# pablomendes/kubeflow-tfx-workshop

Measured on AMD Instinct MI355X. Metric: Trainer examples/sec (whole node), Chicago-Taxi Wide&Deep at 1/2/4/8 MI355X, higher is better.
Workload: dtype bf16; 1 GPU; global_batch=65536, parallelism=dp1, batch_per_gpu=65536, optimizer=adagrad(dnn,lr=0.05)+ftrl(linear,lr=0.2), precision=bf16 MFMA compute, fp32 master weights/optimizer state, device=AMD Radeon Graphics, hipgraph=True, input_shuffle_seed=24301, steps_per_graph=20, kernel=wd_chain (register-chained, 8 waves)

## Files before the change

### csrc/wd_chain.hip

```cpp
#include <hip/hip_runtime.h>
#include "xcd.h"
#include "feed.h"
#include <stdint.h>

namespace {

typedef __bf16 bf16;
typedef __bf16 v8bf __attribute__((ext_vector_type(8)));
typedef __bf16 v4bf __attribute__((ext_vector_type(4)));
typedef __bf16 v2bf __attribute__((ext_vector_type(2)));
typedef short v4s __attribute__((ext_vector_type(4)));
typedef short v8s __attribute__((ext_vector_type(8)));
typedef float v4f __attribute__((ext_vector_type(4)));
typedef __attribute__((address_space(3))) v4s lds_v4s;

#include "wd_opt.h"

#ifndef WDC_T
#define WDC_T 128
#endif
constexpr int T = WDC_T;
static_assert(T == 128 || T == 64 || T == 256, "T");
constexpr bool ONE_ITER = T == 256 || T == 64;
constexpr int MAXW = 8;
constexpr int WPAD = 16;
constexpr int PAD = 8;

constexpr int K1 = 32, N1 = 128;
constexpr int K2 = 128, N2 = 96;
constexpr int K3 = 96, N3 = 64;
constexpr int K4 = 64, N4 = 64;
constexpr int K5 = 64, N5 = 16;

constexpr int LW1 = 0;
constexpr int LW2 = LW1 + N1 * (K1 + WPAD);
constexpr int LW3 = LW2 + N2 * (K2 + WPAD);
constexpr int LW4 = LW3 + N3 * (K3 + WPAD);
constexpr int LW5 = LW4 + N4 * (K4 + WPAD);
constexpr int LWEND = LW5 + N5 * (K5 + WPAD);
constexpr int stage_len(int K, int N) { return T * (N + PAD) + T * (K + PAD); }
constexpr int cmax(int a, int b) { return a > b ? a : b; }
constexpr int WIDE_PAD = 2176;
constexpr bool ROT = T == 256;
constexpr int DMA_GAP = 256;
constexpr int PW2 = ROT ? 0 : LW2;
constexpr int PW3 = PW2 + (LW3 - LW2);
constexpr int PW4 = PW3 + (LW4 - LW3);
constexpr int PW5 = PW4 + (LW5 - LW4);
constexpr int PW1 = ROT ? PW5 + (LWEND - LW5) + DMA_GAP : LW1;
constexpr int PWEND = ROT ? PW1 + (LW2 - LW1) : LWEND;
constexpr int LS = PWEND;
constexpr int SB4 = LS, SB3 = ROT ? PW4 : LS, SB2 = ROT ? PW3 : LS, SB1 = ROT ? PW3 : LS, SB5 = LS;
constexpr int LSEND = cmax(cmax(cmax(SB1 + stage_len(K1, N1), SB2 + stage_len(K2, N2)),
                                cmax(SB3 + stage_len(K3, N3), SB4 + stage_len(K4, N4))),
                           SB5 + stage_len(K5, N5));
// ... 78 lines not shown
__device__ unsigned long long g_wdc_stamps[MAXW][32];
#define STAMP(i)                                                                                  \
  do {                                                                                            \
    __builtin_amdgcn_sched_barrier(0);                                                            \
    if (blockIdx.x == 0 && lane == 0 && stamp_on) g_wdc_stamps[w][i] = __builtin_amdgcn_s_memtime(); \
    __builtin_amdgcn_sched_barrier(0);                                                            \
  } while (0)
__device__ unsigned long long g_wdc_blk[4096][3];
#define BSTAMP(i)                                                                                       \
  do {                                                                                                  \
    __builtin_amdgcn_sched_barrier(0);                                                                  \
    if (w == 0 && lane == 0 && blockIdx.x < 4096) g_wdc_blk[blockIdx.x][i] = __builtin_amdgcn_s_memrealtime(); \
    __builtin_amdgcn_sched_barrier(0);                                                                  \
  } while (0)
#else
#define BSTAMP(i) \
  do {            \
  } while (0)
#define STAMP(i) \
  do {           \
  } while (0)
#endif

template <int K, int N, int TBN>
__device__ __forceinline__ void fwd(const uint16_t* W, const v8bf (&B)[TBN][K / 32], v4f (&acc)[TBN][N / 16], int r,
                                    int h) {
  constexpr int KS = K / 32, NT = N / 16;
#pragma unroll
  for (int nt = 0; nt < NT; ++nt)
#pragma unroll
    for (int tb = 0; tb < TBN; ++tb) acc[tb][nt] = kZero4;
  const int rw[2] = {r, r ^ 4};
  v8bf wa[2][NT];
#pragma unroll
  for (int nt = 0; nt < NT; ++nt) wa[0][nt] = ld8(W + (16 * nt + rw[nt & 1]) * (K + WPAD) + 8 * h);
#pragma unroll
  for (int s = 0; s < KS; ++s) {
    if (s + 1 < KS) {
#pragma unroll
      for (int nt = 0; nt < NT; ++nt) wa[(s + 1) & 1][nt] = ld8(W + (16 * nt + rw[nt & 1]) * (K + WPAD) + 32 * (s + 1) + 8 * h);
    }
#pragma unroll
    for (int nt = 0; nt < NT; ++nt)
#pragma unroll
      for (int tb = 0; tb < TBN; ++tb) acc[tb][nt] = mfma(wa[s & 1][nt], B[tb][s], acc[tb][nt]);
  }
}

template <int N, int TBN>
__device__ __forceinline__ void relu_pack(const v4f (&acc)[TBN][N / 16], v8bf (&out)[TBN][N / 32]) {
#pragma unroll
  for (int tb = 0; tb < TBN; ++tb)
#pragma unroll
    for (int s = 0; s < N / 32; ++s) out[tb][s] = pack_relu(acc[tb][2 * s], acc[tb][2 * s + 1]);
}

template <int K, int N, int TBN>
__device__ __forceinline__ void bwd_dA(const uint16_t* W, const v4bf (&dz)[TBN][N / 16], v4f (&out)[TBN][K / 16], int r,
                                       int h) {
  constexpr int NS = N / 32, KT = K / 16;
  const int q = r >> 2, p = r & 3;
  const int rb = wperm(16 * (h & 1) + 4 * (h >> 1) + q);
  v8bf b[TBN][NS];
#pragma unroll
  for (int tb = 0; tb < TBN; ++tb)
#pragma unroll
    for (int s = 0; s < NS; ++s) b[tb][s] = cat_bf(dz[tb][2 * s], dz[tb][2 * s + 1]);
#pragma unroll
  for (int kt = 0; kt < KT; ++kt)
#pragma unroll
    for (int tb = 0; tb < TBN; ++tb) out[tb][kt] = kZero4;
#pragma unroll
  for (int kt = 0; kt < KT; ++kt) {
    v8bf a[NS];
#pragma unroll
    for (int s = 0; s < NS; ++s) {
      const uint16_t* pa = W + (32 * s + rb) * (K + WPAD) + 16 * kt + 4 * p;
      a[s] = cat8(tr_read(pa), tr_read(pa + 8 * (K + WPAD)));
    }
#pragma unroll
    for (int s = 0; s < NS; ++s)
#pragma unroll
      for (int tb = 0; tb < TBN; ++tb) out[tb][kt] = mfma(a[s], b[tb][s], out[tb][kt]);
  }
}

template <int K, int TBN>
__device__ __forceinline__ void mask_grad(const v4f (&g)[TBN][K / 16], const uint16_t* SA, int w, int r, int h,
                                          v4bf (&dz)[TBN][K / 16]) {
  const int rp = sperm16(r);
#pragma unroll
  for (int tb = 0; tb < TBN; ++tb)
#pragma unroll
    for (int kt = 0; kt < K / 16; ++kt) {
      const int row = 16 * TBN * w + 16 * tb + rp;
      const uint2 m = *(const uint2*)(SA + row * (K + PAD) + 16 * kt + 4 * h);
      const unsigned int u[2] = {mask_pk(cvt_pk(g[tb][kt][0], g[tb][kt][1]), m.x),
                                 mask_pk(cvt_pk(g[tb][kt][2], g[tb][kt][3]), m.y)};
      dz[tb][kt] = __builtin_bit_cast(v4bf, u);
    }
}

template <int K, int N, int TBN>
__device__ __forceinline__ void stage(uint16_t* S, const v4bf (&dz)[TBN][N / 16], const v8bf (&a)[TBN][K / 32], int w,
                                      int r, int h) {
  uint16_t* SZ = S;
  uint16_t* SA = S + T * (N + PAD);
  const int rp = sperm16(r);
#pragma unroll
  for (int tb = 0; tb < TBN; ++tb) {
    const int row = 16 * TBN * w + 16 * tb + rp;
#pragma unroll
    for (int m = 0; m < N / 32; ++m) *(v8bf*)(SZ + row * (N + PAD) + 32 * m + 8 * h) = cat_bf(dz[tb][2 * m], dz[tb][2 * m + 1]);
#pragma unroll
    for (int s = 0; s < K / 32; ++s) *(v8bf*)(SA + row * (K + PAD) + 32 * s + 8 * h) = a[tb][s];
  }
}

template <int K, int N, int NTW, int KTW>
__device__ __forceinline__ void dw_phase(v4f (&acc)[NTW * KTW], const uint16_t* S, int nt0, int ntS, int kt0, int ktS,
                                         int r, int h) {
  const uint16_t* SZ = S;
  const uint16_t* SA = S + T * (N + PAD);
  const int q = r >> 2, p = r & 3;
  const int rl = 16 * (h >> 1) + 8 * (h & 1) + 2 * q;
#pragma unroll
  for (int ts = 0; ts < T / 32; ++ts) {
    v8bf fa[NTW], fb[KTW];
#pragma unroll
    for (int i = 0; i < NTW; ++i) {
      const uint16_t* pa = SZ + (32 * ts + rl) * (N + PAD) + 16 * (nt0 + i * ntS) + 4 * p;
      fa[i] = cat8(tr_read(pa), tr_read(pa + (N + PAD)));
    }
#pragma unroll
    for (int j = 0; j < KTW; ++j) {
      const uint16_t* pb = SA + (32 * ts + rl) * (K + PAD) + 16 * (kt0 + j * ktS) + 4 * p;
      fb[j] = cat8(tr_read(pb), tr_read(pb + (K + PAD)));
    }
#pragma unroll
    for (int i = 0; i < NTW; ++i)
#pragma unroll
      for (int j = 0; j < KTW; ++j) acc[i * KTW + j] = mfma(fa[i], fb[j], acc[i * KTW + j]);
  }
}

template <int K, int NTW, int KTW>
__device__ __forceinline__ void load_ct(int (&ct)[NTW * KTW], int tbase, int nt0, int ntS, int kt0, int ktS,
                                        const int* __restrict__ tmap) {
#pragma unroll
  for (int i = 0; i < NTW; ++i)
#pragma unroll
    for (int j = 0; j < KTW; ++j) ct[i * KTW + j] = tmap[tbase + (nt0 + i * ntS) * (K / 16) + kt0 + j * ktS];
}


#ifndef WDC_NT_SLAB
#define WDC_NT_SLAB 0
#endif
template <class V>
__device__ __forceinline__ void slab_store(V* p, V v) {
  if constexpr (WDC_NT_SLAB) __builtin_nontemporal_store(v, p);
  else *p = v;
}

template <int NT>
__device__ __forceinline__ void store_tiles(float* slab, const v4f (&acc)[NT], const int (&ct)[NT], int lane) {
#pragma unroll
  for (int i = 0; i < NT; ++i) {
    if (ct[i] < 0) continue;
    float* dst = slab + (size_t)ct[i] * 256 + lane;
#pragma unroll
    for (int e = 0; e < 4; ++e) slab_store(dst + e * 64, acc[i][e]);
  }
}

// ... 199 lines not shown
  const long long step0 = (step_ctr && !WDC_DIAG_NOSTEP) ? step_ctr[0] : 0;
  constexpr bool kPersist = PERSIST;
  const int nsteps = kPersist ? ta.nsteps : 1;
  for (int ps = 0; ps < nsteps; ++ps) {
  MifxFeed fd = feed;
  MifxFeedStep fs;
  if (step_ctr) {
    fs = mifx_feed_step(fd, step0 + ps, n_data);
  } else {
    fd.key = 0;
    fs.e0 = 0;
    fs.i0 = start_fixed;
    fs.h = 1;
  }
  const int niters = (int)((batch + T - 1) / T);
  const int my_iters = (niters - (int)blockIdx.x + (int)gridDim.x - 1) / (int)gridDim.x;
  const float qbound = fmaxf(fabsf(grad_scale) * (float)(max(my_iters, 1) * T), 1e-30f);
  const float qscale = exp2f(fminf(floorf(log2f(1073741824.f / qbound)), 100.f));
  const float qinv = 1.f / qscale;
  const float qmax = 1073741824.f / (float)(max(my_iters, 1) * T);

  constexpr bool W4 = NWAVE == 4;
  static_assert(NWAVE == 4 || NWAVE == 8, "waves");
  constexpr int O1N = W4 ? 2 : 1, O2N = W4 ? 6 : 3, O2K = 2, O3K = W4 ? 6 : 3, O4K = W4 ? 4 : 2;
  const int n1 = W4 ? 2 * w : w, n2 = W4 ? 0 : 3 * (w & 1), k2 = W4 ? 2 * w : 2 * (w >> 1),
            n3 = w & 3, k3 = W4 ? 0 : 3 * (w >> 2), n4 = w & 3, k4 = W4 ? 0 : 2 * (w >> 2);
  const bool l5 = w < 4;
  v4f acc1[O1N], acc2[O2N * O2K], acc3[O3K], acc4[O4K], acc5[1];
  int ct1[O1N], ct2[O2N * O2K], ct3[O3K], ct4[O4K], ct5[1];
  if (TRAIN) {
#pragma unroll
    for (int i = 0; i < O1N; ++i) acc1[i] = kZero4;
#pragma unroll
    for (int i = 0; i < O2N * O2K; ++i) acc2[i] = kZero4;
#pragma unroll
    for (int i = 0; i < O3K; ++i) acc3[i] = kZero4;
#pragma unroll
    for (int i = 0; i < O4K; ++i) acc4[i] = kZero4;
    acc5[0] = kZero4;
    load_ct<K1, O1N, 1>(ct1, TB1, n1, 1, 0, 0, tmap);
    load_ct<K2, O2N, O2K>(ct2, TB2, n2, 1, k2, 1, tmap);
    load_ct<K3, 1, O3K>(ct3, TB3, n3, 0, k3, 1, tmap);
    load_ct<K4, 1, O4K>(ct4, TB4, n4, 0, k4, 1, tmap);
    load_ct<K5, 1, 1>(ct5, TB5, 0, 0, w & 3, 0, tmap);
    if (!l5) ct5[0] = -1;
  }
  float loss_sum = 0.f, dl_sum = 0.f;
  const int mtb = TBN == 2 ? (h & 1) : 0;

  auto fetch = [&](int it, uint4 (&u)[TBN][2]) {
#pragma unroll
    for (int tb = 0; tb < TBN; ++tb) {
      const long long row = min((long long)it * T + EPW * w + 16 * tb + r, batch - 1);
      const long long di = mifx_feed_record(fd, fs, row, n_data);
      u[tb][0] = data[2 * di];
      u[tb][1] = data[2 * di + 1];
    }
  };
  uint4 nu[TBN][2];
  fetch(blockIdx.x, nu);
  if constexpr (REG_STAGE) {
#pragma unroll
    for (int i = 0; i < PER_STAGE; ++i)
      if (i * NTHR + tid < NCH_STAGE) *(uint4*)(lds + img_lds((i * NTHR + tid) * 8)) = wst[i];
  }
  if constexpr (!PERSIST) {
    asm volatile("s_waitcnt vmcnt(0)" ::: "memory");
    __syncthreads();
// ... 28 lines not shown
    const uint4 m0 = mtb ? u[TBN - 1][0] : u[0][0], m1 = mtb ? u[TBN - 1][1] : u[0][1];
    const uint32_t idw[5] = {m0.w, m1.x, m1.y, m1.z, m1.w};
    int ids[9];
    float wv[9];
#pragma unroll
    for (int f = 0; f < 9; ++f) {
      int id = (f & 1) ? (idw[f >> 1] >> 16) : (idw[f >> 1] & 0xffff);
      id = id < kWideNb[f] ? id : 0;
      ids[f] = kWideOff[f] + id;
      wv[f] = PERSIST ? wlds[ids[f]] : wide[ids[f]];
    }
    const float wbias = PERSIST ? wlds[WIDE_BIAS] : wide[WIDE_BIAS];

    v8bf a0[TBN][1];
#pragma unroll
    for (int tb = 0; tb < TBN; ++tb) {
      const v8bf x = {(bf16)__uint_as_float(u[tb][0].x), (bf16)__uint_as_float(u[tb][0].y),
                      (bf16)__uint_as_float(u[tb][0].z), (bf16)1.0f, (bf16)0.f, (bf16)0.f, (bf16)0.f, (bf16)0.f};
      a0[tb][0] = h == 0 ? x : (v8bf){};
    }
    v8bf a1[TBN][N1 / 32], a2[TBN][N2 / 32], a3[TBN][N3 / 32], a4[TBN][N4 / 32];
    v4f z5[TBN][1];
    {
      v4f acc[TBN][N1 / 16];
      fwd<K1, N1, TBN>(lds + PW1, a0, acc, r, h);
      relu_pack<N1, TBN>(acc, a1);
    }
    {
      v4f acc[TBN][N2 / 16];
      fwd<K2, N2, TBN>(lds + PW2, a1, acc, r, h);
      relu_pack<N2, TBN>(acc, a2);
    }
    {
      v4f acc[TBN][N3 / 16];
      fwd<K3, N3, TBN>(lds + PW3, a2, acc, r, h);
      relu_pack<N3, TBN>(acc, a3);
    }
    {
      v4f acc[TBN][N4 / 16];
      fwd<K4, N4, TBN>(lds + PW4, a3, acc, r, h);
      relu_pack<N4, TBN>(acc, a4);
    }
    fwd<K5, N5, TBN>(lds + PW5, a4, z5, r, h);

    STAMP(3);
    const float zd0 = __shfl(z5[0][0][0], r), zd1 = __shfl(z5[TBN - 1][0][0], r);
    float wl = wbias;
#pragma unroll
    for (int f = 0; f < 9; ++f) wl += wv[f];
    const float x = (mtb ? zd1 : zd0) + wl;
    const long long grow = (long long)it * T + EPW * w + 16 * mtb + r;
    const bool own = h < TBN && grow < batch;
    const float y = (float)(idw[4] >> 16);
    const float lossv = fmaxf(x, 0.f) - x * y + log1pf(__expf(-fabsf(x)));
    if (!TRAIN) {
      if (own) {
        logits_out[grow] = x;
        loss_sum += lossv;
      }
      continue;
    }
    const float dl = own ? (1.f / (1.f + __expf(-x)) - y) * grad_scale : 0.f;
    if (own) {
      loss_sum += lossv;
      dl_sum += dl;
    }
// ... 16 lines not shown
    }
    {
      v4bf d5[TBN][1];
#pragma unroll
      for (int tb = 0; tb < TBN; ++tb) {
        v4bf o = {(bf16)0.f, (bf16)0.f, (bf16)0.f, (bf16)0.f};
        if (h == 0) o[0] = (bf16)dlb[tb];
        d5[tb][0] = o;
      }
#pragma unroll
      for (int tb = 0; tb < TBN; ++tb) {
        const int row = EPW * w + 16 * tb + sperm16(r);
        *(v4bf*)(S5 + row * (N5 + PAD) + 4 * h) = d5[tb][0];
#pragma unroll
        for (int s = 0; s < K5 / 32; ++s)
          *(v8bf*)(S5 + T * (N5 + PAD) + row * (K5 + PAD) + 32 * s + 8 * h) = a4[tb][s];
      }
    }
    v4bf dz4[TBN][K5 / 16];
    {
      v4f g[TBN][K5 / 16];
#pragma unroll
      for (int kt = 0; kt < K5 / 16; ++kt) {
        const uint2 wv2 = *(const uint2*)(lds + PW5 + 16 * kt + 4 * h);
        const float w5[4] = {__uint_as_float(wv2.x << 16), __uint_as_float(wv2.x & 0xffff0000u),
                             __uint_as_float(wv2.y << 16), __uint_as_float(wv2.y & 0xffff0000u)};
#pragma unroll
        for (int tb = 0; tb < TBN; ++tb)
#pragma unroll
          for (int e = 0; e < 4; ++e) g[tb][kt][e] = w5[e] * dlb[tb];
      }
      mask_grad<K5, TBN>(g, S5 + T * (N5 + PAD), w, r, h, dz4);
    }
    block_sync_lds();
    STAMP(6);
    if (l5) dw_phase<K5, N5, 1, 1>(acc5, S5, 0, 0, w & 3, 0, r, h);
    WDC_EMIT(1, acc5, ct5);
    block_sync_lds();

    STAMP(7);
    stage<K4, N4, TBN>(S4, dz4, a3, w, r, h);
    v4bf dz3[TBN][K4 / 16];
    {
      v4f g[TBN][K4 / 16];
      bwd_dA<K4, N4, TBN>(lds + PW4, dz4, g, r, h);
      mask_grad<K4, TBN>(g, S4 + T * (N4 + PAD), w, r, h, dz3);
    }
    block_sync_lds();
    STAMP(8);
    dw_phase<K4, N4, 1, O4K>(acc4, S4, n4, 0, k4, 1, r, h);
    WDC_EMIT(O4K, acc4, ct4);
    block_sync_lds();

    STAMP(9);
    stage<K3, N3, TBN>(S3, dz3, a2, w, r, h);
    v4bf dz2[TBN][K3 / 16];
    {
      v4f g[TBN][K3 / 16];
      bwd_dA<K3, N3, TBN>(lds + PW3, dz3, g, r, h);
      mask_grad<K3, TBN>(g, S3 + T * (N3 + PAD), w, r, h, dz2);
    }
    block_sync_lds();
    STAMP(10);
    dw_phase<K3, N3, 1, O3K>(acc3, S3, n3, 0, k3, 1, r, h);
    WDC_EMIT(O3K, acc3, ct3);
    block_sync_lds();

    STAMP(11);
    stage<K2, N2, TBN>(S2, dz2, a1, w, r, h);
    v4bf dz1[TBN][K2 / 16];
    {
      v4f g[TBN][K2 / 16];
      bwd_dA<K2, N2, TBN>(lds + PW2, dz2, g, r, h);
      mask_grad<K2, TBN>(g, S2 + T * (N2 + PAD), w, r, h, dz1);
    }
    block_sync_lds();
    STAMP(12);
    dw_phase<K2, N2, O2N, O2K>(acc2, S2, n2, 1, k2, 1, r, h);
    WDC_EMIT(O2N * O2K, acc2, ct2);
    block_sync_lds();

    STAMP(13);
    stage<K1, N1, TBN>(S1, dz1, a0, w, r, h);
    block_sync_lds();
    STAMP(14);
    dw_phase<K1, N1, O1N, 1>(acc1, S1, n1, 1, 0, 0, r, h);
    WDC_EMIT(O1N, acc1, ct1);
    if constexpr (PERSIST) {
      constexpr int NA = O1N + O2N * O2K + O3K + O4K + 1;
      int cta[NA];
#pragma unroll
      for (int i = 0; i < O1N; ++i) cta[i] = ct1[i];
#pragma unroll
      for (int i = 0; i < O2N * O2K; ++i) cta[O1N + i] = ct2[i];
#pragma unroll
      for (int i = 0; i < O3K; ++i) cta[O1N + O2N * O2K + i] = ct3[i];
#pragma unroll
      for (int i = 0; i < O4K; ++i) cta[O1N + O2N * O2K + O3K + i] = ct4[i];
      cta[NA - 1] = ct5[0];
      opt_tiles<NA>(cta, lane, ta, pstep, plast, lds, my_slab);
    }
    STAMP(15);
  }
#ifdef WDC_STAMPS
  stamp_on = true;
#endif
  STAMP(16);

  for (int o = 32; o > 0; o >>= 1) {
    loss_sum += __shfl_xor(loss_sum, o);
    dl_sum += __shfl_xor(dl_sum, o);
  }
  __syncthreads();
  if (lane == 0) {
    red[w] = loss_sum;
    red[NWAVE + w] = dl_sum;
  }
  __syncthreads();
  if constexpr (TRAIN && PERSIST) {
    const bool s1_live = ta.hw.kind >= 2;
    const int w0 = stride - WIDE_PAD;
    for (int c = tid; c < WIDE_PAD; c += NTHR) {
      float v = (float)wgi[c] * qinv;
      wgi[c] = 0;
      if (c == WIDE_BIAS) {
#pragma unroll
        for (int i = 0; i < NWAVE; ++i) v += red[NWAVE + i];
      }
      if (ta.wsc[w0 + c] == -1) continue;
      float a0 = ta.s0[w0 + c], a1 = s1_live ? ta.s1[w0 + c] : 0.f;
      const float nw = opt_update(ta.hw, wlds[c], v, a0, a1, step0 + ps + 1);
      wlds[c] = nw;
      ta.param[w0 + c] = nw;
      ta.s0[w0 + c] = a0;
      if (s1_live) ta.s1[w0 + c] = a1;
    }
  } else if (TRAIN) {
    static_assert(WIDE_PAD % 4 == 0 && (LSEND * 2) % 16 == 0, "vector wide-gradient epilogue");
    v4f* my4 = (v4f*)(slab + (size_t)blockIdx.x * stride + (stride - WIDE_PAD));
    const int4* wgi4 = (const int4*)wgi;
    for (int c4 = tid; c4 < WIDE_PAD / 4; c4 += NTHR) {
      const int4 qv = wgi4[c4];
      float4 v = make_float4((float)qv.x * qinv, (float)qv.y * qinv, (float)qv.z * qinv, (float)qv.w * qinv);
      static_assert(WIDE_BIAS % 4 == 3, "bias column is the .w lane of its float4");
      if (c4 == WIDE_BIAS / 4) {
#pragma unroll
        for (int i = 0; i < NWAVE; ++i) v.w += red[NWAVE + i];
      }
      slab_store(my4 + c4, v4f{v.x, v.y, v.z, v.w});
    }
  }
  if (tid == 0 && slab_loss) {
    float l = 0.f;
#pragma unroll
    for (int i = 0; i < NWAVE; ++i) l += red[i];
    slab_loss[blockIdx.x] = l;
  }
  if constexpr (PERSIST) {
    __builtin_amdgcn_fence(__ATOMIC_RELEASE, "workgroup");
    asm volatile("s_waitcnt vmcnt(0)" ::: "memory");
    __syncthreads();
    __builtin_amdgcn_fence(__ATOMIC_ACQUIRE, "agent");
  }
  }
  if constexpr (PERSIST) {
    for (int i = tid; i < STEP_SLOTS; i += NTHR) ta.step_slots[i] = step0 + nsteps;
  }
  STAMP(17);
  BSTAMP(2);
  if constexpr (TRAIN && TAIL) {
    if (ta.helpers > 0) {
      asm volatile("s_waitcnt vmcnt(0)" ::: "memory");
      __syncthreads();
      if (tid == 0) {
// ... 111 lines not shown
  if (!attr_done) {
    (void)hipFuncSetAttribute((const void*)wdc_fused<TRAIN, TBN, TAIL, PERSIST>,
                              hipFuncAttributeMaxDynamicSharedMemorySize, lds_bytes);
    attr_done = true;
  }
  hipLaunchKernelGGL((wdc_fused<TRAIN, TBN, TAIL, PERSIST>), grid, dim3(64 * (T / (16 * TBN))), lds_bytes, stream,
                     (const uint4*)data, n_data, batch, start_fixed, step_ctr, (const uint4*)wimg, wide, slab,
                     slab_loss, logits_out, grad_scale, tmap, stride, xcd_of, ta, feed);
}

}

#if WDC_T == 128
#define WDC_SYM(n) n
#elif WDC_T == 64
#define WDC_SYM(n) n##_t64
#else
#define WDC_SYM(n) n##_t256
#endif

extern "C" {

int WDC_SYM(mifx_wdc_constants)(int* out, int n) {
  const int v[] = {T, LWEND, LDS_BYTES, WPAD, NTILE, WIDE_PAD, LW1, LW2, LW3, LW4, LW5};
  const int m = (int)(sizeof(v) / sizeof(int));
  for (int i = 0; i < n && i < m; ++i) out[i] = v[i];
  return m;
}

int WDC_SYM(mifx_wdc_fused_f)(const void* data, long long n_data, long long batch, long long start_fixed,
                              const long long* step_ctr, const void* wimg, const float* wide, float* slab,
                              float* slab_loss, float* logits_out, float grad_scale, int grid, int train,
                              const int* tmap, int stride, int waves, int* xcd_of, long long feed_stride,
                              long long feed_offset, unsigned long long shuffle_key, hipStream_t stream) {
  if (grid <= 0 || n_data <= 0 || batch <= 0 || batch > n_data || wimg == nullptr || wide == nullptr) return -1;
  if ((uintptr_t)wimg % 16 != 0 || (uintptr_t)data % 16 != 0) return -1;
  if (train && (tmap == nullptr || slab == nullptr || stride < WIDE_PAD || stride % 4 != 0)) return -1;
  if (!train && logits_out == nullptr) return -1;
  if (feed_stride < batch || feed_offset < 0 || feed_offset + batch > feed_stride) return -1;
  const MifxFeed fd{feed_stride, feed_offset, shuffle_key};
  const dim3 g(grid);
#if WDC_T == 64
  if (waves != 4) return -1;
  if ((long long)grid * T < batch) return -1;
  if (train)
    launch<true, 1>(g, stream, data, n_data, batch, start_fixed, step_ctr, wimg, wide, slab, slab_loss, logits_out,
                    grad_scale, tmap, stride, xcd_of, fd);
// ... 161 lines not shown
```

### mifx/models/wide_deep.py

```python
from __future__ import annotations

import math
from dataclasses import dataclass, field

import numpy as np
import torch
from torch import nn

DENSE_FLOAT_FEATURE_KEYS = ["trip_miles", "fare", "trip_seconds"]
VOCAB_FEATURE_KEYS = ["payment_type", "company"]
BUCKET_FEATURE_KEYS = ["pickup_latitude", "pickup_longitude", "dropoff_latitude", "dropoff_longitude"]
CATEGORICAL_FEATURE_KEYS = [
    "trip_start_hour", "trip_start_day", "trip_start_month", "pickup_census_tract",
    "dropoff_census_tract", "pickup_community_area", "dropoff_community_area",
]
MAX_CATEGORICAL_FEATURE_VALUES = [24, 31, 12]
VOCAB_SIZE = 1000
OOV_SIZE = 10
FEATURE_BUCKET_COUNT = 10
LABEL_KEY = "tips"
FARE_KEY = "fare"


def transformed_name(key: str) -> str:
# ... 242 lines not shown
    rec["id"] = np.clip(np.asarray(ids), 0, 65535).astype(np.uint16)
    rec["label"] = np.asarray(label).astype(np.uint16)
    return rec


CHAIN_PAD = 16
CHAIN_LW = [int(v) for v in np.cumsum([0] + [n * (k + CHAIN_PAD) for k, n in LAYER_KN])[:-1]]
CHAIN_LWEND = sum(n * (k + CHAIN_PAD) for k, n in LAYER_KN)


def chain_perm(K: int) -> np.ndarray:
    c = np.arange(K)
    return 32 * (c // 32) + 16 * ((c % 8) // 4) + 4 * ((c % 32) // 8) + c % 4


def chain_wperm(n: np.ndarray) -> np.ndarray:
    return n ^ (((n >> 4) & 1) << 2)


def chain_dw_rows(li: int) -> np.ndarray:
    N = LAYER_KN[li][1]
    if li == len(LAYER_KN) - 1:
        return np.arange(N)
    c = chain_perm(N)
    return c[c]


def chain_image_offsets(li: int) -> np.ndarray:
    K, N = LAYER_KN[li]
    n = np.arange(N)[:, None]
    c = np.arange(K)[None, :]
    return CHAIN_LW[li] + chain_wperm(n) * (K + CHAIN_PAD) + c


def chain_image(param) -> np.ndarray:
    p = np.asarray(param.detach().cpu() if torch.is_tensor(param) else param, dtype=np.float32)
    img = np.zeros(CHAIN_LWEND, np.float32)
    for li, (K, N) in enumerate(LAYER_KN):
        w = p[LAYER_OFF[li]:LAYER_OFF[li] + K * N].reshape(N, K)
        img[chain_image_offsets(li)] = w[:, chain_perm(K)]
    return img


def chain_maps(cfg: WideDeepConfig | None = None):
    cfg = cfg or WideDeepConfig()
    check_fused_compatible(cfg)
    masks = _trainable_masks(cfg)
    tmap = np.full(NTILE, -1, np.int32)
# ... 28 lines not shown
```

### mifx/ops/wd_chain.py

```python
from __future__ import annotations

import ctypes
import functools

import torch

from . import _lib
from ._lib import F32, I32, I64, U64, VP, check, ptr, sig, stream_handle


HELP_SIG = [VP, I64, I64, VP, VP, VP, VP, VP, F32, VP, I32, VP, VP, VP, VP, VP, VP, VP, VP, I32, I64, I64, U64, VP]


@functools.lru_cache(maxsize=None)
def _fns():
    lib = _lib.load("wd_chain")
    return {
        "constants": sig(lib, "mifx_wdc_constants", [VP, I32]),
        "fused": sig(lib, "mifx_wdc_fused", [VP, I64, I64, I64, VP, VP, VP, VP, VP, VP, F32, I32, I32, VP, I32, I32,
                                             VP]),
        "fused_x": sig(lib, "mifx_wdc_fused_x", [VP, I64, I64, I64, VP, VP, VP, VP, VP, VP, F32, I32, I32, VP, I32,
                                                 I32, VP, VP]),
        "fused_f": sig(lib, "mifx_wdc_fused_f", [VP, I64, I64, I64, VP, VP, VP, VP, VP, VP, F32, I32, I32, VP, I32,
                                                 I32, VP, I64, I64, U64, VP]),
# ... 16 lines not shown
                                                     I32, I32, VP, VP]),
        "fused_f": sig(lib, "mifx_wdc_fused_f_t64", [VP, I64, I64, I64, VP, VP, VP, VP, VP, VP, F32, I32, I32, VP,
                                                     I32, I32, VP, I64, I64, U64, VP]),
        "help": sig(lib, "mifx_wdc_fused_help_t64", HELP_SIG),
    }


@functools.lru_cache(maxsize=None)
def _fns256():
    lib = _lib.load("wd_chain256")
    return {
        "constants": sig(lib, "mifx_wdc_constants_t256", [VP, I32]),
        "fused_f": sig(lib, "mifx_wdc_fused_f_t256", [VP, I64, I64, I64, VP, VP, VP, VP, VP, VP, F32, I32, I32, VP,
                                                      I32, I32, VP, I64, I64, U64, VP]),
    }


def fns_for(tile: int) -> dict:
    if tile not in (64, 128, 256):
        raise ValueError("tile must be 64, 128 or 256")
    return {128: _fns, 64: _fns64, 256: _fns256}[tile]()


@functools.lru_cache(maxsize=None)
def constants() -> dict[str, int]:
    buf = (ctypes.c_int * 16)()
    n = _fns()["constants"](buf, 16)
    names = ["T", "LWEND", "LDS_BYTES", "PAD", "NTILE", "WIDE_PAD", "LW1", "LW2", "LW3", "LW4", "LW5"]
    return {k: buf[i] for i, k in enumerate(names[:n])}


def fused(records: torch.Tensor, n_data: int, batch: int, start_fixed: int, step_ctr: torch.Tensor | None,
          wimg_bf16: torch.Tensor, wide: torch.Tensor, slab: torch.Tensor | None, slab_loss: torch.Tensor | None,
          logits_out: torch.Tensor | None, grad_scale: float, grid: int, train: bool,
          tmap: torch.Tensor | None = None, waves: int = 8, xcd_of: torch.Tensor | None = None,
          tile: int = 128, feed: tuple[int, int, int] | None = None) -> None:
    if waves not in {128: (4, 8), 64: (4,), 256: (8,)}[tile]:
        raise ValueError("waves must be 4 or 8 (tile 128) / 4 (tile 64) / 8 (tile 256)")
    if tile == 256 and train and grid * 256 < batch:
        raise ValueError("tile 256 runs one iteration per workgroup: grid * 256 >= batch")
    c = constants()
    if wimg_bf16.numel() != c["LWEND"] or wimg_bf16.element_size() != 2 or not wimg_bf16.is_contiguous():
        raise ValueError("weight image must be a contiguous 16-bit [LWEND] tensor")
    if records.dim() != 2 or records.shape[1] != 32 or not records.is_contiguous():
        raise ValueError("records must be contiguous uint8 [N, 32]")
    stride = int(slab.shape[-1]) if slab is not None else 0
    if train:
        if tmap is None or tmap.dtype != torch.int32 or tmap.numel() != c["NTILE"]:
            raise ValueError("training launch needs the int32 tile map of the chained slab layout")
        if slab.shape[0] < grid or not slab.is_contiguous():
            raise ValueError("slab must be a contiguous [>= grid, stride] tensor")
        if slab_loss is not None and slab_loss.numel() < grid:
# ... 85 lines not shown
```

### mifx/trainer/fused_wide_deep.py

```python
from __future__ import annotations

import math
from dataclasses import dataclass

import os

import numpy as np
import torch

from ..models import wide_deep as wdm
from ..ops import wide_deep as wdk

OPT_KIND = {"sgd": 0, "adagrad": 1, "ftrl": 2, "adam": 3}


@dataclass
class OptSpec:
    kind: str = "adagrad"
    lr: float = 0.05
    beta1: float = 0.9
    beta2: float = 0.999
    eps: float = 1e-8
    l1: float = 0.0
    l2: float = 0.0
# ... 103 lines not shown
        self.step_ctr = torch.zeros(wdk.STEP_SLOTS, dtype=torch.int64, device=dev)
        self.slab = torch.empty(self.grid, self.stride, device=dev)
        use_xcd = os.environ.get("MIFX_WD_XCD", "1") != "0"
        red_cls = wdk.ResReduce if os.environ.get("MIFX_WD_RES", "1") == "1" and self.world == 1 else wdk.XcdReduce
        self._xcd = red_cls(self.stride, dev) if use_xcd and self._sc and 64 <= self.grid <= 256 else None
        if in_kernel_tail is None:
            in_kernel_tail = os.environ.get("MIFX_WD_TAIL", "0") == "1"
        self._ktail = None
        if in_kernel_tail and self._sc and self.world == 1 and 64 <= self.grid <= 256 and self.waves == 8 \
                and self.device.type == "cuda" and self.grid <= torch.cuda.get_device_properties(dev).multi_processor_count:
            from ..ops import wd_chain as wdc

            self._ktail = wdc.InKernelTail(self.stride, dev)
        if persistent is None:
            persistent = os.environ.get("MIFX_WD_PERSIST", "0") == "1"
        self._persist = bool(persistent and self._sc and self.world == 1 and self.grid == 1 and self.batch <= self.T
                             and self.waves == 8 and self._ktail is None and self.device.type == "cuda")
        if small_tile is None:
            small_tile = os.environ.get("MIFX_WD_T64", "1") == "1"
        self.tile = 256 if self._t256 else 64 if (small_tile and kernel == "chain" and self.batch <= 64 and self.grid == 1
                                                  and not self._persist and self._ktail is None) else 128
        if self.tile == 64:
            self.waves = 4
        if one_launch is None:
            one_launch = os.environ.get("MIFX_WD_ONE_LAUNCH", "0") == "1"
        self._one = None
        if one_launch and self._sc and self.world == 1 and self.grid == 1 and self.fused_update \
                and not self._persist and self._ktail is None and self.device.type == "cuda" \
                and (self.tile == 64 or (self.tile == 128 and self.waves == 8)):
            from ..ops import wd_chain as wdc

            self._one = wdc.OneRowTail(self.stride, self.tile, dev)
        self.slab_loss = torch.zeros(self.grid, device=dev)
        self.nsplit = max(1, min(16, self.grid // 8))
        self.partial = torch.empty(self.nsplit, self.stride, device=dev)
        self.grad = torch.empty(1, self.stride, device=dev)
        self.h_dnn = self.dnn_opt.encode()
        self.h_wide = self.wide_opt.encode()
        self.records = None
        self.n_data = 0
        self.graph = None
        self._graphs = None
        self._fast = None
        self._direct = None
        self._xg = None
        self.graph_multi, self.graph_multi_steps = None, 1
# ... 339 lines not shown
```

Measured before the change: 2.466 billion examples/s.

## Skip padded zero tiles in chained Wide&Deep forward, backward and dW MFMAs

After: 2.537 billion examples/s, median of 6. +2.9%, better.

```diff
diff --git a/csrc/wd_chain.hip b/csrc/wd_chain.hip
--- a/csrc/wd_chain.hip
+++ b/csrc/wd_chain.hip
@@ -31,6 +31,20 @@
 constexpr int K3 = 96, N3 = 64;
 constexpr int K4 = 64, N4 = 64;
 constexpr int K5 = 64, N5 = 16;
+constexpr int R0 = 3, R1 = 100, R2 = 70, R3 = 48, R4 = 34, R5 = 1;
+constexpr int cdiv16(int n) { return (n + 15) / 16; }
+constexpr int live_ctiles(int live, int K) {
+  int n = 0;
+  for (int t = 0; t < K / 16; ++t) n += 32 * (t / 2) + 8 * (t % 2) < live ? 1 : 0;
+  return n;
+}
+constexpr int FN1 = cdiv16(R1 + 1), FN2 = cdiv16(R2 + 1), FN3 = cdiv16(R3 + 1), FN4 = cdiv16(R4 + 1), FN5 = cdiv16(R5);
+constexpr int DN1 = cdiv16(R1), DN2 = cdiv16(R2), DN3 = cdiv16(R3), DN4 = cdiv16(R4), DN5 = cdiv16(R5);
+constexpr int KT1 = live_ctiles(R0 + 1, K1), KT2 = live_ctiles(R1 + 1, K2), KT3 = live_ctiles(R2 + 1, K3),
+              KT4 = live_ctiles(R3 + 1, K4), KT5 = live_ctiles(R4 + 1, K5);
+static_assert(FN1 == 7 && FN2 == 5 && FN3 == 4 && FN4 == 3 && FN5 == 1, "forward n tiles");
+static_assert(KT1 == 1 && KT2 == 7 && KT3 == 5 && KT4 == 4 && KT5 == 3, "C-order k tiles");
+static_assert(DN1 * KT1 + DN2 * KT2 + DN3 * KT3 + DN4 * KT4 + DN5 * KT5 == 72, "live dW tiles");
 
 constexpr int LW1 = 0;
 constexpr int LW2 = LW1 + N1 * (K1 + WPAD);
@@ -155,10 +169,10 @@
   } while (0)
 #endif
 
-template <int K, int N, int TBN>
-__device__ __forceinline__ void fwd(const uint16_t* W, const v8bf (&B)[TBN][K / 32], v4f (&acc)[TBN][N / 16], int r,
+template <int K, int NT, int TBN>
+__device__ __forceinline__ void fwd(const uint16_t* W, const v8bf (&B)[TBN][K / 32], v4f (&acc)[TBN][NT], int r,
                                     int h) {
-  constexpr int KS = K / 32, NT = N / 16;
+  constexpr int KS = K / 32;
 #pragma unroll
   for (int nt = 0; nt < NT; ++nt)
 #pragma unroll
@@ -180,18 +194,28 @@
   }
 }
 
-template <int N, int TBN>
-__device__ __forceinline__ void relu_pack(const v4f (&acc)[TBN][N / 16], v8bf (&out)[TBN][N / 32]) {
+template <int N, int NT, int TBN>
+__device__ __forceinline__ void relu_pack(const v4f (&acc)[TBN][NT], v8bf (&out)[TBN][N / 32]) {
 #pragma unroll
   for (int tb = 0; tb < TBN; ++tb)
 #pragma unroll
-    for (int s = 0; s < N / 32; ++s) out[tb][s] = pack_relu(acc[tb][2 * s], acc[tb][2 * s + 1]);
-}
-
-template <int K, int N, int TBN>
+    for (int s = 0; s < N / 32; ++s) {
+      if (2 * s + 1 < NT) {
+        out[tb][s] = pack_relu(acc[tb][2 * s], acc[tb][2 * s + 1]);
+      } else if (2 * s < NT) {
+        const unsigned int u[4] = {relu_pk(cvt_pk(acc[tb][2 * s][0], acc[tb][2 * s][1])),
+                                   relu_pk(cvt_pk(acc[tb][2 * s][2], acc[tb][2 * s][3])), 0u, 0u};
+        out[tb][s] = __builtin_bit_cast(v8bf, u);
+      } else {
+        out[tb][s] = (v8bf){};
+      }
+    }
+}
+
+template <int K, int N, int KTL, int NTL, int TBN>
 __device__ __forceinline__ void bwd_dA(const uint16_t* W, const v4bf (&dz)[TBN][N / 16], v4f (&out)[TBN][K / 16], int r,
                                        int h) {
-  constexpr int NS = N / 32, KT = K / 16;
+  constexpr int NS = (NTL + 1) / 2, KT = K / 16;
   const int q = r >> 2, p = r & 3;
   const int rb = wperm(16 * (h & 1) + 4 * (h >> 1) + q);
   v8bf b[TBN][NS];
@@ -204,7 +228,7 @@
 #pragma unroll
     for (int tb = 0; tb < TBN; ++tb) out[tb][kt] = kZero4;
 #pragma unroll
-  for (int kt = 0; kt < KT; ++kt) {
+  for (int kt = 0; kt < KTL; ++kt) {
     v8bf a[NS];
 #pragma unroll
     for (int s = 0; s < NS; ++s) {
@@ -218,7 +242,7 @@
   }
 }
 
-template <int K, int TBN>
+template <int K, int KTL, int TBN>
 __device__ __forceinline__ void mask_grad(const v4f (&g)[TBN][K / 16], const uint16_t* SA, int w, int r, int h,
                                           v4bf (&dz)[TBN][K / 16]) {
   const int rp = sperm16(r);
@@ -226,6 +250,10 @@
   for (int tb = 0; tb < TBN; ++tb)
 #pragma unroll
     for (int kt = 0; kt < K / 16; ++kt) {
+      if (kt >= KTL) {
+        dz[tb][kt] = (v4bf){(bf16)0.f, (bf16)0.f, (bf16)0.f, (bf16)0.f};
+        continue;
+      }
       const int row = 16 * TBN * w + 16 * tb + rp;
       const uint2 m = *(const uint2*)(SA + row * (K + PAD) + 16 * kt + 4 * h);
       const unsigned int u[2] = {mask_pk(cvt_pk(g[tb][kt][0], g[tb][kt][1]), m.x),
@@ -240,50 +268,69 @@
   uint16_t* SZ = S;
   uint16_t* SA = S + T * (N + PAD);
   const int rp = sperm16(r);
+  const int hz = 2 * (h & 1) + (h >> 1);
 #pragma unroll
   for (int tb = 0; tb < TBN; ++tb) {
     const int row = 16 * TBN * w + 16 * tb + rp;
 #pragma unroll
-    for (int m = 0; m < N / 32; ++m) *(v8bf*)(SZ + row * (N + PAD) + 32 * m + 8 * h) = cat_bf(dz[tb][2 * m], dz[tb][2 * m + 1]);
+    for (int m = 0; m < N / 32; ++m) *(v8bf*)(SZ + row * (N + PAD) + 32 * m + 8 * hz) = cat_bf(dz[tb][2 * m], dz[tb][2 * m + 1]);
 #pragma unroll
     for (int s = 0; s < K / 32; ++s) *(v8bf*)(SA + row * (K + PAD) + 32 * s + 8 * h) = a[tb][s];
   }
 }
 
-template <int K, int N, int NTW, int KTW>
+template <int K, int N, int NTW, int KTW, int NA = NTW, int KA = KTW>
 __device__ __forceinline__ void dw_phase(v4f (&acc)[NTW * KTW], const uint16_t* S, int nt0, int ntS, int kt0, int ktS,
                                          int r, int h) {
+  static_assert(NA >= 1 && NA <= NTW && KA >= 1 && KA <= KTW, "live part of the block");
   const uint16_t* SZ = S;
   const uint16_t* SA = S + T * (N + PAD);
   const int q = r >> 2, p = r & 3;
   const int rl = 16 * (h >> 1) + 8 * (h & 1) + 2 * q;
 #pragma unroll
   for (int ts = 0; ts < T / 32; ++ts) {
-    v8bf fa[NTW], fb[KTW];
-#pragma unroll
-    for (int i = 0; i < NTW; ++i) {
+    v8bf fa[NA], fb[KA];
+#pragma unroll
+    for (int i = 0; i < NA; ++i) {
       const uint16_t* pa = SZ + (32 * ts + rl) * (N + PAD) + 16 * (nt0 + i * ntS) + 4 * p;
       fa[i] = cat8(tr_read(pa), tr_read(pa + (N + PAD)));
     }
 #pragma unroll
-    for (int j = 0; j < KTW; ++j) {
+    for (int j = 0; j < KA; ++j) {
       const uint16_t* pb = SA + (32 * ts + rl) * (K + PAD) + 16 * (kt0 + j * ktS) + 4 * p;
       fb[j] = cat8(tr_read(pb), tr_read(pb + (K + PAD)));
     }
 #pragma unroll
-    for (int i = 0; i < NTW; ++i)
-#pragma unroll
-      for (int j = 0; j < KTW; ++j) acc[i * KTW + j] = mfma(fa[i], fb[j], acc[i * KTW + j]);
+    for (int i = 0; i < NA; ++i)
+#pragma unroll
+      for (int j = 0; j < KA; ++j) acc[i * KTW + j] = mfma(fa[i], fb[j], acc[i * KTW + j]);
+  }
+}
+
+template <int K, int N, int NTW, int KTW, int NA0, int NA1, int KA0, int KA1>
+__device__ __forceinline__ void dw_phase_sel(v4f (&acc)[NTW * KTW], const uint16_t* S, int nt0, int kt0, bool nsel,
+                                             bool ksel, int r, int h) {
+  const bool n1 = NA0 != NA1 && nsel, k1 = KA0 != KA1 && ksel;
+  if (!n1) {
+    if (!k1) dw_phase<K, N, NTW, KTW, NA0, KA0>(acc, S, nt0, 1, kt0, 1, r, h);
+    else dw_phase<K, N, NTW, KTW, NA0, KA1>(acc, S, nt0, 1, kt0, 1, r, h);
+  } else {
+    if (!k1) dw_phase<K, N, NTW, KTW, NA1, KA0>(acc, S, nt0, 1, kt0, 1, r, h);
+    else dw_phase<K, N, NTW, KTW, NA1, KA1>(acc, S, nt0, 1, kt0, 1, r, h);
   }
 }
 
 template <int K, int NTW, int KTW>
-__device__ __forceinline__ void load_ct(int (&ct)[NTW * KTW], int tbase, int nt0, int ntS, int kt0, int ktS,
+__device__ __forceinline__ void load_ct(int (&ct)[NTW * KTW], int tbase, int nt0, int na, int kt0, int ka,
                                         const int* __restrict__ tmap) {
 #pragma unroll
   for (int i = 0; i < NTW; ++i)
 #pragma unroll
-    for (int j = 0; j < KTW; ++j) ct[i * KTW + j] = tmap[tbase + (nt0 + i * ntS) * (K / 16) + kt0 + j * ktS];
+    for (int j = 0; j < KTW; ++j) {
+      const bool own = i < na && j < ka;
+      const int v = tmap[own ? tbase + (nt0 + i) * (K / 16) + kt0 + j : 0];
+      ct[i * KTW + j] = own ? v : -1;
+    }
 }
 
 
@@ -529,10 +576,17 @@
 
   constexpr bool W4 = NWAVE == 4;
   static_assert(NWAVE == 4 || NWAVE == 8, "waves");
-  constexpr int O1N = W4 ? 2 : 1, O2N = W4 ? 6 : 3, O2K = 2, O3K = W4 ? 6 : 3, O4K = W4 ? 4 : 2;
+  static_assert(DN1 == 7 && DN2 == 5 && KT2 == 7 && DN3 == 3 && KT3 == 5 && DN4 == 3 && KT4 == 4 && DN5 == 1 &&
+                KT5 == 3 && KT1 == 1, "the ownership below is written for these live tiles");
+  constexpr int O1N = W4 ? 2 : 1, O2N = W4 ? DN2 : 3, O2K = 2, O3K = W4 ? KT3 : 3, O4K = W4 ? KT4 : 2;
+  const int wu = __builtin_amdgcn_readfirstlane(w);
   const int n1 = W4 ? 2 * w : w, n2 = W4 ? 0 : 3 * (w & 1), k2 = W4 ? 2 * w : 2 * (w >> 1),
-            n3 = w & 3, k3 = W4 ? 0 : 3 * (w >> 2), n4 = w & 3, k4 = W4 ? 0 : 2 * (w >> 2);
-  const bool l5 = w < 4;
+            n3 = W4 ? w : w % 3, k3 = W4 ? 0 : 3 * (w / 3), n4 = W4 ? w : w % 3, k4 = W4 ? 0 : 2 * (w / 3);
+  const int na1 = W4 ? (wu < 3 ? 2 : 1) : (wu < DN1 ? 1 : 0);
+  const int na2 = W4 ? DN2 : ((wu & 1) ? 2 : 3), ka2 = (W4 ? wu : wu >> 1) < 3 ? 2 : 1;
+  const int na3 = W4 ? (wu < DN3 ? 1 : 0) : (wu < 6 ? 1 : 0), ka3 = W4 ? KT3 : (wu < 3 ? 3 : 2);
+  const int na4 = W4 ? (wu < DN4 ? 1 : 0) : (wu < 6 ? 1 : 0), ka4 = W4 ? KT4 : 2;
+  const bool l5 = wu < KT5;
   v4f acc1[O1N], acc2[O2N * O2K], acc3[O3K], acc4[O4K], acc5[1];
   int ct1[O1N], ct2[O2N * O2K], ct3[O3K], ct4[O4K], ct5[1];
   if (TRAIN) {
@@ -545,12 +599,11 @@
 #pragma unroll
     for (int i = 0; i < O4K; ++i) acc4[i] = kZero4;
     acc5[0] = kZero4;
-    load_ct<K1, O1N, 1>(ct1, TB1, n1, 1, 0, 0, tmap);
-    load_ct<K2, O2N, O2K>(ct2, TB2, n2, 1, k2, 1, tmap);
-    load_ct<K3, 1, O3K>(ct3, TB3, n3, 0, k3, 1, tmap);
-    load_ct<K4, 1, O4K>(ct4, TB4, n4, 0, k4, 1, tmap);
-    load_ct<K5, 1, 1>(ct5, TB5, 0, 0, w & 3, 0, tmap);
-    if (!l5) ct5[0] = -1;
+    load_ct<K1, O1N, 1>(ct1, TB1, n1, na1, 0, 1, tmap);
+    load_ct<K2, O2N, O2K>(ct2, TB2, n2, na2, k2, ka2, tmap);
+    load_ct<K3, 1, O3K>(ct3, TB3, n3, na3, k3, ka3, tmap);
+    load_ct<K4, 1, O4K>(ct4, TB4, n4, na4, k4, ka4, tmap);
+    load_ct<K5, 1, 1>(ct5, TB5, 0, 1, w & 3, l5 ? 1 : 0, tmap);
   }
   float loss_sum = 0.f, dl_sum = 0.f;
   const int mtb = TBN == 2 ? (h & 1) : 0;
@@ -625,26 +678,26 @@
     v8bf a1[TBN][N1 / 32], a2[TBN][N2 / 32], a3[TBN][N3 / 32], a4[TBN][N4 / 32];
     v4f z5[TBN][1];
     {
-      v4f acc[TBN][N1 / 16];
-      fwd<K1, N1, TBN>(lds + PW1, a0, acc, r, h);
-      relu_pack<N1, TBN>(acc, a1);
+      v4f acc[TBN][FN1];
+      fwd<K1, FN1, TBN>(lds + PW1, a0, acc, r, h);
+      relu_pack<N1, FN1, TBN>(acc, a1);
     }
     {
-      v4f acc[TBN][N2 / 16];
-      fwd<K2, N2, TBN>(lds + PW2, a1, acc, r, h);
-      relu_pack<N2, TBN>(acc, a2);
+      v4f acc[TBN][FN2];
+      fwd<K2, FN2, TBN>(lds + PW2, a1, acc, r, h);
+      relu_pack<N2, FN2, TBN>(acc, a2);
     }
     {
-      v4f acc[TBN][N3 / 16];
-      fwd<K3, N3, TBN>(lds + PW3, a2, acc, r, h);
-      relu_pack<N3, TBN>(acc, a3);
+      v4f acc[TBN][FN3];
+      fwd<K3, FN3, TBN>(lds + PW3, a2, acc, r, h);
+      relu_pack<N3, FN3, TBN>(acc, a3);
     }
     {
-      v4f acc[TBN][N4 / 16];
-      fwd<K4, N4, TBN>(lds + PW4, a3, acc, r, h);
-      relu_pack<N4, TBN>(acc, a4);
-    }
-    fwd<K5, N5, TBN>(lds + PW5, a4, z5, r, h);
+      v4f acc[TBN][FN4];
+      fwd<K4, FN4, TBN>(lds + PW4, a3, acc, r, h);
+      relu_pack<N4, FN4, TBN>(acc, a4);
+    }
+    fwd<K5, FN5, TBN>(lds + PW5, a4, z5, r, h);
 
     STAMP(3);
     const float zd0 = __shfl(z5[0][0][0], r), zd1 = __shfl(z5[TBN - 1][0][0], r);
@@ -707,6 +760,11 @@
       v4f g[TBN][K5 / 16];
 #pragma unroll
       for (int kt = 0; kt < K5 / 16; ++kt) {
+        if (kt >= KT5) {
+#pragma unroll
+          for (int tb = 0; tb < TBN; ++tb) g[tb][kt] = kZero4;
+          continue;
+        }
         const uint2 wv2 = *(const uint2*)(lds + PW5 + 16 * kt + 4 * h);
         const float w5[4] = {__uint_as_float(wv2.x << 16), __uint_as_float(wv2.x & 0xffff0000u),
                              __uint_as_float(wv2.y << 16), __uint_as_float(wv2.y & 0xffff0000u)};
@@ -715,7 +773,7 @@
 #pragma unroll
           for (int e = 0; e < 4; ++e) g[tb][kt][e] = w5[e] * dlb[tb];
       }
-      mask_grad<K5, TBN>(g, S5 + T * (N5 + PAD), w, r, h, dz4);
+      mask_grad<K5, KT5, TBN>(g, S5 + T * (N5 + PAD), w, r, h, dz4);
     }
     block_sync_lds();
     STAMP(6);
@@ -728,12 +786,12 @@
     v4bf dz3[TBN][K4 / 16];
     {
       v4f g[TBN][K4 / 16];
-      bwd_dA<K4, N4, TBN>(lds + PW4, dz4, g, r, h);
-      mask_grad<K4, TBN>(g, S4 + T * (N4 + PAD), w, r, h, dz3);
+      bwd_dA<K4, N4, KT4, KT5, TBN>(lds + PW4, dz4, g, r, h);
+      mask_grad<K4, KT4, TBN>(g, S4 + T * (N4 + PAD), w, r, h, dz3);
     }
     block_sync_lds();
     STAMP(8);
-    dw_phase<K4, N4, 1, O4K>(acc4, S4, n4, 0, k4, 1, r, h);
+    if (na4) dw_phase<K4, N4, 1, O4K>(acc4, S4, n4, 0, k4, 1, r, h);
     WDC_EMIT(O4K, acc4, ct4);
     block_sync_lds();
 
@@ -742,12 +800,12 @@
     v4bf dz2[TBN][K3 / 16];
     {
       v4f g[TBN][K3 / 16];
-      bwd_dA<K3, N3, TBN>(lds + PW3, dz3, g, r, h);
-      mask_grad<K3, TBN>(g, S3 + T * (N3 + PAD), w, r, h, dz2);
+      bwd_dA<K3, N3, KT3, KT4, TBN>(lds + PW3, dz3, g, r, h);
+      mask_grad<K3, KT3, TBN>(g, S3 + T * (N3 + PAD), w, r, h, dz2);
     }
     block_sync_lds();
     STAMP(10);
-    dw_phase<K3, N3, 1, O3K>(acc3, S3, n3, 0, k3, 1, r, h);
+    if (na3) dw_phase_sel<K3, N3, 1, O3K, 1, 1, O3K, W4 ? O3K : 2>(acc3, S3, n3, k3, false, ka3 != O3K, r, h);
     WDC_EMIT(O3K, acc3, ct3);
     block_sync_lds();
 
@@ -756,12 +814,12 @@
     v4bf dz1[TBN][K2 / 16];
     {
       v4f g[TBN][K2 / 16];
-      bwd_dA<K2, N2, TBN>(lds + PW2, dz2, g, r, h);
-      mask_grad<K2, TBN>(g, S2 + T * (N2 + PAD), w, r, h, dz1);
+      bwd_dA<K2, N2, KT2, KT3, TBN>(lds + PW2, dz2, g, r, h);
+      mask_grad<K2, KT2, TBN>(g, S2 + T * (N2 + PAD), w, r, h, dz1);
     }
     block_sync_lds();
     STAMP(12);
-    dw_phase<K2, N2, O2N, O2K>(acc2, S2, n2, 1, k2, 1, r, h);
+    dw_phase_sel<K2, N2, O2N, O2K, O2N, W4 ? O2N : 2, O2K, 1>(acc2, S2, n2, k2, na2 != O2N, ka2 != O2K, r, h);
     WDC_EMIT(O2N * O2K, acc2, ct2);
     block_sync_lds();
 
@@ -769,7 +827,7 @@
     stage<K1, N1, TBN>(S1, dz1, a0, w, r, h);
     block_sync_lds();
     STAMP(14);
-    dw_phase<K1, N1, O1N, 1>(acc1, S1, n1, 1, 0, 0, r, h);
+    if (na1) dw_phase_sel<K1, N1, O1N, 1, O1N, 1, 1, 1>(acc1, S1, n1, 0, na1 != O1N, false, r, h);
     WDC_EMIT(O1N, acc1, ct1);
     if constexpr (PERSIST) {
       constexpr int NA = O1N + O2N * O2K + O3K + O4K + 1;
@@ -797,6 +855,7 @@
     dl_sum += __shfl_xor(dl_sum, o);
   }
   __syncthreads();
+  STAMP(18);
   if (lane == 0) {
     red[w] = loss_sum;
     red[NWAVE + w] = dl_sum;
@@ -835,6 +894,7 @@
       slab_store(my4 + c4, v4f{v.x, v.y, v.z, v.w});
     }
   }
+  STAMP(19);
   if (tid == 0 && slab_loss) {
     float l = 0.f;
 #pragma unroll
@@ -992,7 +1052,8 @@
 extern "C" {
 
 int WDC_SYM(mifx_wdc_constants)(int* out, int n) {
-  const int v[] = {T, LWEND, LDS_BYTES, WPAD, NTILE, WIDE_PAD, LW1, LW2, LW3, LW4, LW5};
+  const int v[] = {T,   LWEND, LDS_BYTES, WPAD, NTILE, WIDE_PAD, LW1, LW2, LW3, LW4, LW5, FN1, FN2,
+                   FN3, FN4,   FN5,       DN1,  DN2,   DN3,      DN4, DN5, KT1, KT2, KT3, KT4, KT5};
   const int m = (int)(sizeof(v) / sizeof(int));
   for (int i = 0; i < n && i < m; ++i) out[i] = v[i];
   return m;
diff --git a/mifx/models/wide_deep.py b/mifx/models/wide_deep.py
--- a/mifx/models/wide_deep.py
+++ b/mifx/models/wide_deep.py
@@ -288,8 +288,19 @@
     N = LAYER_KN[li][1]
     if li == len(LAYER_KN) - 1:
         return np.arange(N)
-    c = chain_perm(N)
-    return c[c]
+    j = np.arange(N)
+    return 16 * (j // 16) + 8 * ((j % 8) // 4) + 4 * ((j % 16) // 8) + j % 4
+
+
+def chain_live_tiles(cfg: WideDeepConfig | None = None) -> list[tuple[int, int, int]]:
+    cfg = cfg or WideDeepConfig()
+    out = []
+    for li, ((K, N), (kr, nr)) in enumerate(zip(LAYER_KN, _real_dims(cfg))):
+        last = li == len(LAYER_KN) - 1
+        fn = -(-(nr if last else nr + 1) // 16)
+        kt = sum(1 for t in range(K // 16) if 32 * (t // 2) + 8 * (t % 2) < kr + 1)
+        out.append((fn, -(-nr // 16), kt))
+    return out
 
 
 def chain_image_offsets(li: int) -> np.ndarray:
diff --git a/mifx/ops/wd_chain.py b/mifx/ops/wd_chain.py
--- a/mifx/ops/wd_chain.py
+++ b/mifx/ops/wd_chain.py
@@ -62,12 +62,36 @@
     return {128: _fns, 64: _fns64, 256: _fns256}[tile]()
 
 
-@functools.lru_cache(maxsize=None)
-def constants() -> dict[str, int]:
-    buf = (ctypes.c_int * 16)()
-    n = _fns()["constants"](buf, 16)
-    names = ["T", "LWEND", "LDS_BYTES", "PAD", "NTILE", "WIDE_PAD", "LW1", "LW2", "LW3", "LW4", "LW5"]
-    return {k: buf[i] for i, k in enumerate(names[:n])}
+_CONST_NAMES = ["T", "LWEND", "LDS_BYTES", "PAD", "NTILE", "WIDE_PAD", "LW1", "LW2", "LW3", "LW4", "LW5"] + \
+    [f"{p}{l}" for p in ("FN", "DN", "KT") for l in range(1, 6)]
+
+
+@functools.lru_cache(maxsize=None)
+def constants(tile: int = 128) -> dict[str, int]:
+    buf = (ctypes.c_int * 32)()
+    n = fns_for(tile)["constants"](buf, 32)
+    if n != len(_CONST_NAMES):
+        raise RuntimeError(f"chained W&D kernel (T = {tile}) exports {n} constants, expected {len(_CONST_NAMES)}")
+    return {k: buf[i] for i, k in enumerate(_CONST_NAMES)}
+
+
+def check_live_tiles(cfg, tmap, tile: int) -> None:
+    import numpy as np
+
+    from ..models import wide_deep as wdm
+
+    c = constants(tile)
+    tmap = np.asarray(tmap.cpu() if torch.is_tensor(tmap) else tmap)
+    for li, ((K, N), (fn, dn, kt)) in enumerate(zip(wdm.LAYER_KN, wdm.chain_live_tiles(cfg))):
+        kern = (c[f"FN{li + 1}"], c[f"DN{li + 1}"], c[f"KT{li + 1}"])
+        if kern != (fn, dn, kt):
+            raise ValueError(f"chained W&D kernel (T = {tile}) is compiled for {kern} live (forward n, dW n, k) tiles "
+                             f"in layer {li + 1}; the model has {(fn, dn, kt)}")
+        live = tmap[wdm.TILE_BASE[li]:wdm.TILE_BASE[li] + (N // 16) * (K // 16)].reshape(N // 16, K // 16) >= 0
+        want = (np.arange(N // 16)[:, None] < kern[1]) & (np.arange(K // 16)[None, :] < kern[2])
+        if not np.array_equal(live, want):
+            raise ValueError(f"the tile map's live dW tiles of layer {li + 1} are not the {kern[1]} x {kern[2]} the "
+                             f"chained W&D kernel (T = {tile}) computes")
 
 
 def fused(records: torch.Tensor, n_data: int, batch: int, start_fixed: int, step_ctr: torch.Tensor | None,
diff --git a/mifx/trainer/fused_wide_deep.py b/mifx/trainer/fused_wide_deep.py
--- a/mifx/trainer/fused_wide_deep.py
+++ b/mifx/trainer/fused_wide_deep.py
@@ -149,6 +149,11 @@
                                                   and not self._persist and self._ktail is None) else 128
         if self.tile == 64:
             self.waves = 4
+        if kernel == "chain":
+            from ..ops import wd_chain as wdc
+
+            for t in sorted({128, self.tile}):
+                wdc.check_live_tiles(self.model.cfg, tmap, t)
         if one_launch is None:
             one_launch = os.environ.get("MIFX_WD_ONE_LAUNCH", "0") == "1"
         self._one = None
```
